# 6Lackiu/EMplanner_Carla

Hardware: AMD Instinct MI355X
Metric: planning cycles/sec (DP+QP, 40x9 S-L lattice, 8 obs) (higher is better)
Workload: dtype f64

## Files before the change

emplanner_carla_amd/csrc/emp_api.hip:

```cpp
#include <stdlib.h>
#include <string.h>

#include <algorithm>
#include <tuple>

#include "emp_context.h"
#ifndef EMP_QP_LDS_PAD
#define EMP_QP_LDS_PAD 0
#endif
#ifndef EMP_EDGE_LDS_PAD
#define EMP_EDGE_LDS_PAD 0
#endif
#include "emp_dp_kernels.h"
#include "emp_st_kernels.h"
#include "emp_st_backend_kernels.h"
#include "emp_tail_kernels.h"
#include "emp_mpc_kernels.h"
#include "emp_rollout_kernels.h"
#include "emp_speed_front_kernels.h"
#include "emp_drive_kernels.h"

namespace emp {
thread_local std::string g_create_error;

// ... 818 lines not shown
static bool qp_reserved_ok(const emp_qp_params* q) { return EMP_DEV_HOOKS || q->reserved == 0; }

static QpDev make_qp_dev(const emp_qp_params* q) {
    QpDev d;
    d.qp = PathQpParams{q->ds, q->w_l, q->w_ddl, q->w_dddl, q->w_centre, q->host_d1, q->host_d2, q->host_w};
    d.obs_length = q->obs_length;
    d.obs_width = q->obs_width;
    d.decimate = q->decimate > 0 ? q->decimate : 1;
    d.midpoint = q->midpoint;
    d.use_qp = q->use_qp;
    d.debug_stage = EMP_DEV_HOOKS ? q->reserved : 0;
    return d;
}

static inline dim3 grid1(int n, int block) { return dim3((unsigned)((n + block - 1) / block)); }
static inline dim3 grid_groups(int B, int per_wave) { return grid1(B, per_wave); }

static int dev_project(emp_ctx* ctx, int B, int max_ref, int max_obs, const double* ref_line, const int* n_ref,
                       const double* origin_xy, const double* start_xy, const double* start_v, const double* start_a,
                       const double* obs_xy, const int* n_obs, double* s_map, double* obs_s, double* obs_l,
                       double* begin_sl, double* start, int obs_cap = -1, const double* dyn = nullptr,
                       int* n_obs_out = nullptr) {
    if (B == 0) return EMP_OK;
    const size_t lds = (size_t)7 * max_ref * sizeof(double);
    if (const int rc = set_lds(ctx, frenet_project_wave_kernel, lds, "reference line too long for the LDS-resident projection kernel")) return rc;
    return launch(ctx, "project", frenet_project_wave_kernel, dim3(B), dim3(64), lds, B, max_ref, max_obs, ref_line, n_ref, origin_xy,
                  start_xy, start_v, start_a, obs_xy, n_obs, s_map, obs_s, obs_l, begin_sl, start, obs_cap < 0 ? max_obs : obs_cap, dyn,
                  n_obs_out);
}

template <typename... A>
static int dev_reference_line(emp_ctx* ctx, const emp_smooth_params* sp, int B, int max_global, A... args) {
    if (B == 0) return EMP_OK;
    const SmoothQpParams sx{sp->w_smooth, sp->w_length, sp->w_ref, sp->x_thre};
    const SmoothQpParams sy{sp->w_smooth, sp->w_length, sp->w_ref, sp->y_thre};
    const size_t lds = (2 * (size_t)kRefLinePoints + 2 * (size_t)BoxRangeQp::words(kRefLinePoints, kRefLinePoints) +
                        (size_t)kRefLinePoints) * sizeof(double);
    if (const int rc = set_lds(ctx, reference_line_wave_kernel, lds, kQpTooLarge)) return rc;
    return launch(ctx, "reference_line", reference_line_wave_kernel, dim3(B), dim3(64), lds, B, max_global, sx, sy, args...);
}

static int dev_cycle_qp(emp_ctx* ctx, int B, int max_pts, int max_obs, const QpDev& Q, const double* dp_s,
                        const double* dp_l, const int* dp_len, const double* obs_s, const double* obs_l,
                        const int* n_obs, const double* start, double* path_s, double* path_l, int* path_len,
                        int* status, CycleSched* cs) {
    if (B == 0) return EMP_OK;
    const int cap = (max_pts + Q.decimate - 1) / Q.decimate;
    const size_t per_group = ((size_t)5 * cap + 4 * (size_t)max_obs + path_qp_words(cap)) * sizeof(double);
    int rc;
    KernelTimer t(ctx, "path_qp");
    const bool pair_form = ctx->opt[EMP_OPT_PATH_QP_FORM] == 1;
    if (cap <= 66 && !pair_form) {
        const int gp = cap <= 34 ? 8 : 16;
        const size_t words = cap <= 26 ? cycle_qp_group_words<8, 3>(cap, max_obs) : cap <= 34 ? cycle_qp_group_words<8, 4>(cap, max_obs)
                                                                                                : cycle_qp_group_words<16, 4>(cap, max_obs);
        const size_t per_wave = (size_t)(64 / gp) * words * sizeof(double) + EMP_QP_LDS_PAD;
        auto kern = cap <= 26 ? cycle_qp_rows_kernel<8, 3> : cap <= 34 ? cycle_qp_rows_kernel<8, 4> : cycle_qp_rows_kernel<16, 4>;
        if ((rc = set_lds(ctx, kern, per_wave, kQpTooLarge))) return rc;
        const int spw = 64 / gp;
        return launch_attaching(ctx, cs, t.stop != nullptr, kern, dim3((B + spw - 1) / spw), dim3(64), per_wave, B, max_pts,
                                max_obs, cap, Q, dp_s, dp_l, dp_len, obs_s, obs_l, n_obs, start, path_s, path_l, path_len, status);
    } else if (cap <= 34) {
        const size_t per_pair = 2 * ((size_t)5 * cap + 4 * (size_t)max_obs + path_qp_words_pair()) * sizeof(double);
        auto kern = cycle_qp_wave_kernel<32>;
        if ((rc = set_lds(ctx, kern, per_pair, kQpTooLarge))) return rc;
        return launch_attaching(ctx, cs, t.stop != nullptr, kern, dim3((B + 1) / 2), dim3(64), per_pair, B, max_pts,
                                max_obs, cap, Q, dp_s, dp_l, dp_len, obs_s, obs_l, n_obs, start, path_s, path_l, path_len, status);
    }
    if ((rc = set_lds(ctx, cycle_qp_wave_kernel<64>, per_group, kQpTooLarge))) return rc;
    return launch_attaching(ctx, cs, t.stop != nullptr, cycle_qp_wave_kernel<64>, dim3(B), dim3(64), per_group, B, max_pts, max_obs, cap,
                            Q, dp_s, dp_l, dp_len, obs_s, obs_l, n_obs, start, path_s, path_l, path_len, status);
}

static int dev_cycle_cartesian(emp_ctx* ctx, int B, int max_ref, int max_pts, int path_cap, const emp_smooth_params* sp,
                               const double* ref_line, const double* s_map, const int* n_ref, const double* begin_sl,
                               const double* path_s, const double* path_l, const int* path_len, double* traj,
                               int* traj_len, int* status) {
    if (B == 0) return EMP_OK;
    const SmoothQpParams sx{sp->w_smooth, sp->w_length, sp->w_ref, sp->x_thre};
    const SmoothQpParams sy{sp->w_smooth, sp->w_length, sp->w_ref, sp->y_thre};
    const int cap = path_cap + 1;
    const size_t lds = ((size_t)max_ref + 3 * (size_t)cap + 2 * (size_t)BoxRangeQp::words(cap, cap)) * sizeof(double);
    const bool wave_form = ctx->opt[EMP_OPT_CARTESIAN_FORM] == 1;
    if (cap <= 64 && !wave_form) {
        const int spw = cap <= 32 ? 4 : 2;
        const size_t lds4 = ((size_t)spw * ((size_t)max_ref + 5 * (size_t)cap) + 2 * (size_t)BoxRangeQp::words(cap, cap)) * sizeof(double);
        auto k4 = cap <= 24 ? cycle_cartesian_rows_kernel<8, 3> : cap <= 32 ? cycle_cartesian_rows_kernel<8, 4> : cycle_cartesian_rows_kernel<16, 4>;
        if (const int rc = set_lds(ctx, k4, lds4, kQpTooLarge)) return rc;
        const int force_fb = ctx->opt[EMP_OPT_SMOOTH_FORCE_FALLBACK] ? 1 : 0;
        return launch(ctx, "to_cartesian", k4, dim3((B + spw - 1) / spw), dim3(64), lds4, B, max_ref, max_pts, cap, sx, sy, ref_line,
                      s_map, n_ref, begin_sl, path_s, path_l, path_len, traj, traj_len, status, force_fb);
    }
    auto kern = cap > 32 ? cycle_cartesian_wave_kernel_wide : cycle_cartesian_wave_kernel_narrow;
    if (const int rc = set_lds(ctx, kern, lds, kQpTooLarge)) return rc;
    return launch(ctx, "to_cartesian", kern, dim3(B), dim3(64), lds, B, max_ref, max_pts, cap, sx, sy, ref_line, s_map, n_ref,
                  begin_sl, path_s, path_l, path_len, traj, traj_len, status);
}

class CycleLane {
  public:
    CycleLane(emp_ctx* c, int m, bool p) : ctx(c), mode(m), pinned(p) {}
    ~CycleLane() {
        if (!ln) return;
        ctx->stream = ctx->main_stream;
        std::swap(ctx->pool, ln->pool);
        ctx->active_lane = -1;
    }

    int begin() {
// ... 2000 lines not shown
```

emplanner_carla_amd/csrc/emp_qp_core.h:

```cpp
#pragma once

#include "emp_core.h"

#ifndef EMP_QP_TRACE
#define EMP_QP_TRACE(...)
#endif

namespace emp {

constexpr int kQpMaxIter = 60;
#ifndef EMP_QP_TAU
#define EMP_QP_TAU(mu) fmax(0.99, 1.0 - (mu))
#endif
EMP_HD double qp_step_fraction(double mu) { return EMP_QP_TAU(mu); }
constexpr int kQpStallIter = 16;
constexpr double kQpStallResidual = 1e-3;

template <int KD>
EMP_HD bool band_chol(double* a, int n) {
    constexpr int W = KD + 1;
    for (int i = 0; i < n; ++i) {
        for (int d = 0; d <= KD && i + d < n; ++d) {
            double sum = a[i * W + d];
            const int j = i + d;
// ... 447 lines not shown
            if (i == 0 || i == n - 1) {
                if (v > ub + tol || v < lb - tol) return 1;
            } else {
                const int t = i - 1;
                Q.c[t * 2 + f] = v;
                Q.lo[t * 2 + f] = lb;
                Q.hi[t * 2 + f] = ub;
            }
        }
    }
    const double ds2 = ds * ds;
    const double a[3] = {1.0 / 6.0, 4.0 / 6.0, 1.0 / 6.0};
    const double b[3] = {1.0 / ds2, -2.0 / ds2, 1.0 / ds2};
    const double jk[4] = {-1.0 / ds2, 3.0 / ds2, -3.0 / ds2, 1.0 / ds2};
    const double wl2 = 2.0 * (prm.w_l + prm.w_centre), wd2 = 2.0 * prm.w_ddl, wj2 = 2.0 * prm.w_dddl;
    for (int m = 0; m < N; ++m) {
        Q.q[m] = 0.0;
        Q.u[m] = 0.0;
        for (int d = 0; d < 4; ++d) Q.P[m * 4 + d] = 0.0;
    }
    auto add = [&](int jp, int jq, double val) {
        const int fp = jp - 3, fq = jq - 3;
        const bool pf = fp >= 0 && fp < N, qf = fq >= 0 && fq < N;
        if (pf && qf) Q.P[fp * 4 + (fq - fp)] += val;
        else if (pf) Q.q[fp] += val * cc[jq];
        else if (qf) Q.q[fq] += val * cc[jp];
    };
    for (int i = 0; i < n; ++i) {
        for (int p = 0; p < 3; ++p)
            for (int r = p; r < 3; ++r) add(i + p, i + r, wl2 * a[p] * a[r] + wd2 * b[p] * b[r]);
        if (i + 1 < n)
            for (int p = 0; p < 4; ++p)
                for (int r = p; r < 4; ++r) add(i + p, i + r, wj2 * jk[p] * jk[r]);
        const double lin = -2.0 * prm.w_centre * ((l_min[i] + l_max[i]) / 2.0);
        for (int p = 0; p < 3; ++p) {
            const int f = i + p - 3;
            if (f >= 0 && f < N) Q.q[f] += lin * a[p];
        }
    }
    return 0;
}

EMP_HD void path_qp_finish(const double* cc, int n, double ds, double* out_l, double* out_dl, double* out_ddl) {
    for (int i = 0; i < n; ++i) {
        out_l[i] = (cc[i] + 4.0 * cc[i + 1] + cc[i + 2]) / 6.0;
        if (out_dl) out_dl[i] = (cc[i + 2] - cc[i]) / (2.0 * ds);
        if (out_ddl) out_ddl[i] = (cc[i] - 2.0 * cc[i + 1] + cc[i + 2]) / (ds * ds);
    }
}

EMP_HD constexpr int path_qp_words_pair() { return 36 + PathRangeQp::words_fast(32, 32); }
EMP_HD constexpr int path_qp_words(int n) { return PathRangeQp::words(n - 4 > 0 ? n - 4 : 0, n - 2 > 0 ? n - 2 : 0) + n + 2; }

EMP_HD int path_qp_solve_scalar(double* mem, const double* l_min, const double* l_max, int n, double l0, double dl0,
                                double ddl0, const PathQpParams& prm, double* out_l, double* out_dl, double* out_ddl,
                                int* iters, double* gi_work = nullptr) {
    *iters = 0;
    if (n < 4) return 2;
    PathRangeQp Q;
    double* cc = mem;
    Q.bind(mem + n + 2, n - 4, n - 2);
    int rc = path_qp_setup(Q, cc, l_min, l_max, n, l0, dl0, ddl0, prm);
    if (rc) return rc;
    if (Q.N > 0) {
        for (int m = 0; m < Q.N * 4; ++m) Q.M[m] = Q.P[m];
        if (!band_chol<3>(Q.M, Q.N)) return 2;
        for (int m = 0; m < Q.N; ++m) Q.u[m] = -Q.q[m];
        band_solve<3>(Q.M, Q.u, Q.N);
        rc = gi_work ? range_qp_gi_scalar(Q, gi_work) : Q.solve_scalar();
        *iters = Q.iters;
        if (rc) return rc;
        for (int m = 0; m < Q.N; ++m) cc[m + 3] = Q.u[m];
    } else {
        for (int t = 0; t < Q.ns; ++t)
            for (int f = 0; f < 2; ++f)
                if (Q.c[t * 2 + f] > Q.hi[t * 2 + f] + 1e-9 || Q.c[t * 2 + f] < Q.lo[t * 2 + f] - 1e-9) return 1;
    }
    path_qp_finish(cc, n, prm.ds, out_l, out_dl, out_ddl);
    return 0;
}

struct SmoothQpParams {
    double w_smooth, w_length, w_ref, thr;
};

EMP_HD void box_qp_forms(BoxRangeQp& Q) {
    Q.off0 = 0;
    Q.g[0][0] = 1.0;
    Q.eps_p = 1e-10;
    Q.eps_mu = 1e-13;
    Q.eps_d_rel = 1e-10;
}

EMP_HD int box_qp_setup(BoxRangeQp& Q, const double* ref, int stride, int m, const SmoothQpParams& prm) {
    if (m < 2 || !(prm.thr > 0.0)) return 2;
    box_qp_forms(Q);
    for (int i = 0; i < m * 3; ++i) Q.P[i] = 0.0;
    for (int i = 0; i < m; ++i) Q.P[i * 3] += 2.0 * prm.w_ref;
    const double d2[3] = {1.0, -2.0, 1.0};
    for (int r = 0; r + 2 < m; ++r)
        for (int p = 0; p < 3; ++p)
            for (int cidx = p; cidx < 3; ++cidx) Q.P[(r + p) * 3 + (cidx - p)] += 2.0 * prm.w_smooth * d2[p] * d2[cidx];
    const double d1[2] = {1.0, -1.0};
    for (int r = 0; r + 1 < m; ++r)
        for (int p = 0; p < 2; ++p)
            for (int cidx = p; cidx < 2; ++cidx) Q.P[(r + p) * 3 + (cidx - p)] += 2.0 * prm.w_length * d1[p] * d1[cidx];
// ... 13 lines not shown
```

emplanner_carla_amd/csrc/emp_qp_rows.h:

```cpp
#pragma once

#include "emp_qp_wave.h"

#ifndef EMP_QP_DEBUG_ROWS
#define EMP_QP_DEBUG_ROWS(...)
#endif

namespace emp {

#pragma clang fp contract(fast)

template <int GP, class Op>
__device__ __forceinline__ double oct_reduce(double v, Op op) {
    static_assert(GP == 8 || GP == 16, "groups of 8 or 16 lanes");
    v = op(v, dpp_move<0xB1>(v));
    v = op(v, dpp_move<0x4E>(v));
    v = op(v, dpp_move<0x141>(v));
    if constexpr (GP == 16) v = op(v, dpp_move<0x140>(v));
    return v;
}
template <int GP>
__device__ __forceinline__ double oct_max(double v) { return oct_reduce<GP>(v, [](double a, double b) { return vmax(a, b); }); }
template <int GP>
__device__ __forceinline__ double oct_min(double v) { return oct_reduce<GP>(v, [](double a, double b) { return vmin(a, b); }); }
// ... 110 lines not shown
        for (int r = 0; r < R; ++r) {
            const double y1 = (r >= 1) ? y[r - 1] : p1;
            const double y2 = (r >= 2) ? y[r - 2] : (r == 1 ? p1 : p2);
            const double y3 = (r >= 3) ? y[r - 3] : (r == 2 ? p1 : (r == 1 ? p2 : p3));
            double acc = __builtin_fma(-low[r][1], y1, rhs[r]);
            acc = __builtin_fma(-low[r][2], y2, acc);
            acc = __builtin_fma(-low[r][3], y3, acc);
            y[r] = acc * rinv[r];
        }
    }
    double x[R];
#pragma unroll
    for (int r = 0; r < R; ++r) x[r] = y[r] * rinv[r];
    for (int k = 0; k < steps; ++k) {
        const double q1 = lane_dn1(x[0]), q2 = lane_dn1(x[1]), q3 = lane_dn1(x[2]);
#pragma unroll
        for (int r = R - 1; r >= 0; --r) {
            const double x1 = (r + 1 < R) ? x[r + 1] : q1;
            const double x2 = (r + 2 < R) ? x[r + 2] : (r + 2 == R ? q1 : q2);
            const double x3 = (r + 3 < R) ? x[r + 3] : (r + 3 == R ? q1 : (r + 3 == R + 1 ? q2 : q3));
            double acc = __builtin_fma(-a[r][1], x1, y[r]);
            acc = __builtin_fma(-a[r][2], x2, acc);
            acc = __builtin_fma(-a[r][3], x3, acc);
            x[r] = acc * rinv[r];
        }
    }
#pragma unroll
    for (int r = 0; r < R; ++r) b[r] = x[r];
}

template <int GP, int R>
__device__ int path_qp_solve_rows(PathRangeQp& Q, int gl, bool live, int iter_cap, double* keep) {
    constexpr int F = 2, W = 3;
    const int N = Q.N, ns = Q.ns, rows = ns * F * 2;
    int state = (live && N > 0) ? 1 : 0;
    int iters = 0;
    bool acceptable = false;
    const int base = gl * R;
    const int steps = oct_wave_max<GP>((state == 1) ? (N + R - 1) / R : 0);
    double g[F][W], gg0[W][F], gg1[W - 1][F], gg2[W - 2][F];
#pragma unroll
    for (int f = 0; f < F; ++f) {
#pragma unroll
        for (int p = 0; p < W; ++p) g[f][p] = wave_uniform(Q.g[f][p]);
    }
#pragma unroll
    for (int f = 0; f < F; ++f) {
#pragma unroll
        for (int p = 0; p < W; ++p) gg0[p][f] = wave_uniform(g[f][p] * g[f][p]);
#pragma unroll
        for (int p = 0; p < W - 1; ++p) gg1[p][f] = wave_uniform(g[f][p] * g[f][p + 1]);
        gg2[0][f] = wave_uniform(g[f][0] * g[f][2]);
    }
    unsigned tmask = 0, mmask = 0, uwm = 0, swm = 0, uxm = 0;
#pragma unroll
    for (int r = 0; r < R; ++r) {
        if (live && base + r < ns) tmask |= 1u << r;
        if (live && base + r < N) mmask |= 1u << r;
    }
#pragma unroll
    for (int i = 0; i < R + 2; ++i) {
        const int k = base - 2 + i;
        if (live && k >= 0 && k < N) uwm |= 1u << i;
        if (live && base + i < ns) swm |= 1u << i;
    }
#pragma unroll
    for (int i = 0; i < R + 6; ++i) {
        const int k = base - 3 + i;
        if (live && k >= 0 && k < N) uxm |= 1u << i;
    }
    auto ld = [](const double* a, int i, bool ok) {
        const double raw = a[i];
        return ok ? raw : 0.0;
    };
    auto win = [&](const double* vec, double (&out)[R][F]) {
        double vals[R + 2];
#pragma unroll
        for (int i = 0; i < R + 2; ++i) vals[i] = ld(vec, base - 2 + i, (uwm >> i) & 1u);
#pragma unroll
        for (int r = 0; r < R; ++r) {
#pragma unroll
            for (int f = 0; f < F; ++f) out[r][f] = (g[f][0] * vals[r] + g[f][1] * vals[r + 1]) + g[f][2] * vals[r + 2];
        }
    };
    auto gather = [&](const double* coef, double (&out)[R]) {
        double cw[R + 2][F];
#pragma unroll
        for (int i = 0; i < R + 2; ++i) {
#pragma unroll
            for (int f = 0; f < F; ++f) cw[i][f] = ld(coef, (base + i) * F + f, (swm >> i) & 1u);
        }
#pragma unroll
        for (int r = 0; r < R; ++r) {
            double acc = 0.0;
#pragma unroll
            for (int p = 0; p < W; ++p) {
#pragma unroll
                for (int f = 0; f < F; ++f) acc += g[f][p] * cw[r + 2 - p][f];
            }
            out[r] = acc;
        }
    };
    auto bounds = [&](double (&c_it)[R][F], double (&lo_it)[R][F], double (&hi_it)[R][F]) {
#pragma unroll
        for (int r = 0; r < R; ++r) {
            const bool ok = (tmask >> r) & 1u;
#pragma unroll
            for (int f = 0; f < F; ++f) {
                const double c = Q.c[(base + r) * F + f], lo = Q.lo[(base + r) * F + f], hi = Q.hi[(base + r) * F + f];
                c_it[r][f] = ok ? c : 0.0;
                lo_it[r][f] = ok ? lo : -1e300;
                hi_it[r][f] = ok ? hi : 1e300;
            }
        }
    };

    double su[R][F], sl[R][F], zu[R][F], zl[R][F];
    double pdiag = 0.0, qabs = 0.0;
#pragma unroll
    for (int r = 0; r < R; ++r) {
        const bool ok = (mmask >> r) & 1u;
        pdiag = fmax(pdiag, ld(Q.P, (base + r) * 4, ok));
        qabs = fmax(qabs, fabs(ld(Q.q, base + r, ok)));
    }
    const double pscale = oct_max<GP>(pdiag);
    const double qscale = fmax(oct_max<GP>(qabs), 1.0);
    {
        const double z0 = Q.initial_multiplier(pscale);
        double v[R][F], c_it[R][F], lo_it[R][F], hi_it[R][F];
        bounds(c_it, lo_it, hi_it);
        win(Q.u, v);
        double smin = 1e300;
#pragma unroll
        for (int r = 0; r < R; ++r) {
#pragma unroll
            for (int f = 0; f < F; ++f) {
                zu[r][f] = zl[r][f] = z0;
                su[r][f] = hi_it[r][f] - (c_it[r][f] + v[r][f]);
                sl[r][f] = (c_it[r][f] + v[r][f]) - lo_it[r][f];
                if ((tmask >> r) & 1u) smin = fmin(smin, fmin(su[r][f], sl[r][f]));
            }
        }
        smin = oct_min<GP>(smin);
        const double shift = (smin < 1.0) ? (1.0 - smin) : 0.0;
#pragma unroll
        for (int r = 0; r < R; ++r) {
#pragma unroll
            for (int f = 0; f < F; ++f) {
                su[r][f] += shift;
                sl[r][f] += shift;
            }
        }
    }

    bool restore = false;
    while (__any(state == 1)) {
        const bool run = state == 1;
        bool acc_now = false;
        double rpu[R][F], rpl[R][F], isu[R][F], isl[R][F], izu[R][F], izl[R][F];
        double rp_max = 0.0, zmax = 0.0, mu = 0.0;
        {
            double v[R][F], c_it[R][F], lo_it[R][F], hi_it[R][F];
            bounds(c_it, lo_it, hi_it);
            win(Q.u, v);
#pragma unroll
            for (int r = 0; r < R; ++r) {
                const bool ok = run && ((tmask >> r) & 1u);
#pragma unroll
                for (int f = 0; f < F; ++f) {
                    rpu[r][f] = (c_it[r][f] + v[r][f]) - hi_it[r][f] + su[r][f];
                    rpl[r][f] = lo_it[r][f] - (c_it[r][f] + v[r][f]) + sl[r][f];
                    isu[r][f] = fast_rcp(su[r][f]);
                    isl[r][f] = fast_rcp(sl[r][f]);
                    izu[r][f] = fast_rcp(zu[r][f]);
                    izl[r][f] = fast_rcp(zl[r][f]);
                    if (ok) {
                        Q.tmp[(base + r) * F + f] = zu[r][f] - zl[r][f];
                        Q.wgt[(base + r) * F + f] = zu[r][f] * isu[r][f] + zl[r][f] * isl[r][f];
                        rp_max = vmax(rp_max, vmax_abs(rpu[r][f], rpl[r][f]));
                        zmax = vmax(zmax, vmax(zu[r][f], zl[r][f]));
                        mu += su[r][f] * zu[r][f] + sl[r][f] * zl[r][f];
                    }
                }
            }
        }
        __syncthreads();
        double rd_m[R], fa[R][4], flow[R][4], frinv[R];
        {
            double ux[R + 6], gz[R];
#pragma unroll
            for (int i = 0; i < R + 6; ++i) ux[i] = ld(Q.u, base - 3 + i, (uxm >> i) & 1u);
            gather(Q.tmp, gz);
            double ww[R + 2][F];
#pragma unroll
            for (int i = 0; i < R + 2; ++i) {
#pragma unroll
                for (int f = 0; f < F; ++f) ww[i][f] = ld(Q.wgt, (base + i) * F + f, (swm >> i) & 1u);
            }
            double rd_max = 0.0;
#pragma unroll
            for (int r = 0; r < R; ++r) {
                const bool ok = run && ((mmask >> r) & 1u);
                const int m = base + r;
                double acc = Q.q[m];
#pragma unroll
                for (int d = 0; d < 4; ++d) acc += Q.P[m * 4 + d] * ux[r + 3 + d];
#pragma unroll
                for (int d = 1; d < 4; ++d) acc += ld(Q.P, (m - d) * 4 + d, m - d >= 0) * ux[r + 3 - d];
                rd_m[r] = ok ? acc + gz[r] : 0.0;
                rd_max = vmax_abs(rd_max, rd_m[r]);
                double e0 = Q.P[m * 4 + 0], e1 = Q.P[m * 4 + 1], e2 = Q.P[m * 4 + 2];
                const double e3 = Q.P[m * 4 + 3];
#pragma unroll
                for (int f = 0; f < F; ++f) {
                    e0 += (ww[r + 2][f] * gg0[0][f] + ww[r + 1][f] * gg0[1][f]) + ww[r][f] * gg0[2][f];
                    e1 += ww[r + 2][f] * gg1[0][f] + ww[r + 1][f] * gg1[1][f];
                    e2 += ww[r + 2][f] * gg2[0][f];
                }
                fa[r][0] = ok ? e0 : 0.0;
                fa[r][1] = (ok && m + 1 < N) ? e1 : 0.0;
                fa[r][2] = (ok && m + 2 < N) ? e2 : 0.0;
                fa[r][3] = (ok && m + 3 < N) ? e3 : 0.0;
            }
            rd_max = oct_max<GP>(rd_max);
            rp_max = oct_max<GP>(rp_max);
            zmax = oct_max<GP>(zmax);
            mu = oct_sum<GP>(mu) / (double)rows;
            if (run) {
                const double dscale = fmax(qscale, zmax);
                if (rd_max <= Q.eps_d_rel * dscale && rp_max <= Q.eps_p && mu <= Q.eps_mu) state = 0;
                else if (!(mu == mu) || mu > 1e30 || (iters >= kQpStallIter && rp_max > kQpStallResidual)) state = 2;
                else if (rp_max > kQpStallResidual && zmax > kQpInfeasibleZ * pscale) state = 2;
                else if (iters >= kQpMaxIter || iters >= iter_cap) state = acceptable ? 0 : 2;
                acc_now = rd_max <= 100.0 * Q.eps_d_rel * dscale && rp_max <= 10.0 * Q.eps_p && mu <= 1000.0 * Q.eps_mu;
                if (acc_now) acceptable = true;
                if (state == 1 && acc_now && rp_max <= Q.eps_p && mu <= Q.eps_mu) state = 0;
                if (state == 0 && acceptable && !acc_now) restore = true;
                EMP_QP_DEBUG_ROWS("R it %d rd %.3e rp %.3e mu %.3e zmax %.3e -> state %d acc %d\n", iters, rd_max, rp_max, mu, zmax, state, (int)acceptable);
            }
        }
        if (run && acc_now) {
#pragma unroll
            for (int r = 0; r < R; ++r)
                if ((mmask >> r) & 1u) keep[base + r] = Q.u[base + r];
        }
        if (!__any(state == 1)) break;
        const bool go = state == 1;
#ifdef EMP_QP_PROBE_SKIP_CHOL
        bool okf = true;
#pragma unroll
        for (int r = 0; r < R; ++r) {
            frinv[r] = 1.0 / (fa[r][0] + 1.0);
#pragma unroll
            for (int d = 0; d < 4; ++d) flow[r][d] = 0.0;
        }
#else
        const bool okf = band_chol_rows<GP, R>(fa, frinv, flow, N, gl, go, steps);
#endif
        EMP_QP_DEBUG_ROWS("R    chol ok %d\n", (int)okf);
        if (go && !okf) {
            state = acceptable ? 0 : 2;
            if (acceptable && !acc_now) restore = true;
        }
        const bool go2 = state == 1;
#pragma unroll
        for (int r = 0; r < R; ++r) {
            if (go2 && ((tmask >> r) & 1u)) {
#pragma unroll
                for (int f = 0; f < F; ++f)
                    Q.tmp[(base + r) * F + f] = -(((zu[r][f] * isu[r][f]) * rpu[r][f] - zu[r][f]) - ((zl[r][f] * isl[r][f]) * rpl[r][f] - zl[r][f]));
            }
        }
        __syncthreads();
        double dua[R];
        gather(Q.tmp, dua);
#pragma unroll
        for (int r = 0; r < R; ++r) dua[r] = (go2 && ((mmask >> r) & 1u)) ? (-rd_m[r] + dua[r]) : 0.0;
#ifndef EMP_QP_PROBE_SKIP_SOLVE
        band_solve_rows<R>(fa, frinv, flow, dua, steps);
#endif
#pragma unroll
        for (int r = 0; r < R; ++r)
            if (go2 && ((mmask >> r) & 1u)) Q.dua[base + r] = dua[r];
        __syncthreads();
        double rcu[R][F], rcl[R][F];
        {
            double gda[R][F], dsua[R][F], dsla[R][F], dzua[R][F], dzla[R][F];
            win(Q.dua, gda);
            double ratio = 0.0;
#pragma unroll
            for (int r = 0; r < R; ++r) {
                const bool ok = go2 && ((tmask >> r) & 1u);
#pragma unroll
                for (int f = 0; f < F; ++f) {
                    dsua[r][f] = -rpu[r][f] - gda[r][f];
                    dsla[r][f] = -rpl[r][f] + gda[r][f];
                    dzua[r][f] = -zu[r][f] - (zu[r][f] * isu[r][f]) * dsua[r][f];
                    dzla[r][f] = -zl[r][f] - (zl[r][f] * isl[r][f]) * dsla[r][f];
                    if (ok)
                        ratio = vmax(ratio, vmax(vmax(-dsua[r][f] * isu[r][f], -dsla[r][f] * isl[r][f]),
                                                 vmax(-dzua[r][f] * izu[r][f], -dzla[r][f] * izl[r][f])));
                }
            }
            ratio = oct_max<GP>(ratio);
            const double a_aff = (ratio > 1.0) ? fast_rcp(ratio) : 1.0;
            double mu_aff = 0.0;
#pragma unroll
            for (int r = 0; r < R; ++r) {
                if (go2 && ((tmask >> r) & 1u)) {
#pragma unroll
                    for (int f = 0; f < F; ++f)
                        mu_aff += (su[r][f] + a_aff * dsua[r][f]) * (zu[r][f] + a_aff * dzua[r][f]) +
                                  (sl[r][f] + a_aff * dsla[r][f]) * (zl[r][f] + a_aff * dzla[r][f]);
                }
            }
            mu_aff = oct_sum<GP>(mu_aff) / (double)rows;
            double sigma = (mu > 0.0) ? mu_aff * fast_rcp(mu) : 0.0;
            sigma = sigma * sigma * sigma;
#pragma unroll
            for (int r = 0; r < R; ++r) {
                const bool ok = go2 && ((tmask >> r) & 1u);
#pragma unroll
                for (int f = 0; f < F; ++f) {
                    rcu[r][f] = su[r][f] * zu[r][f] + dsua[r][f] * dzua[r][f] - sigma * mu;
                    rcl[r][f] = sl[r][f] * zl[r][f] + dsla[r][f] * dzla[r][f] - sigma * mu;
                }
                if (ok) {
#pragma unroll
                    for (int f = 0; f < F; ++f)
                        Q.tmp[(base + r) * F + f] = -((zu[r][f] * rpu[r][f] - rcu[r][f]) * isu[r][f] - (zl[r][f] * rpl[r][f] - rcl[r][f]) * isl[r][f]);
                }
            }
        }
        __syncthreads();
        double du[R];
        gather(Q.tmp, du);
#pragma unroll
        for (int r = 0; r < R; ++r) du[r] = (go2 && ((mmask >> r) & 1u)) ? (-rd_m[r] + du[r]) : 0.0;
#ifndef EMP_QP_PROBE_SKIP_SOLVE
        band_solve_rows<R>(fa, frinv, flow, du, steps);
#endif
#pragma unroll
        for (int r = 0; r < R; ++r)
            if (go2 && ((mmask >> r) & 1u)) Q.rhs[base + r] = du[r];
        __syncthreads();
        {
            double gd[R][F], dsu[R][F], dsl[R][F], dzu[R][F], dzl[R][F];
            win(Q.rhs, gd);
            double ratio = 0.0;
#pragma unroll
            for (int r = 0; r < R; ++r) {
                const bool ok = go2 && ((tmask >> r) & 1u);
#pragma unroll
                for (int f = 0; f < F; ++f) {
                    dsu[r][f] = -rpu[r][f] - gd[r][f];
                    dsl[r][f] = -rpl[r][f] + gd[r][f];
                    dzu[r][f] = -(rcu[r][f] + zu[r][f] * dsu[r][f]) * isu[r][f];
                    dzl[r][f] = -(rcl[r][f] + zl[r][f] * dsl[r][f]) * isl[r][f];
                    if (ok)
                        ratio = vmax(ratio, vmax(vmax(-dsu[r][f] * isu[r][f], -dsl[r][f] * isl[r][f]),
                                                 vmax(-dzu[r][f] * izu[r][f], -dzl[r][f] * izl[r][f])));
                }
            }
            ratio = oct_max<GP>(ratio);
            const double tau = qp_step_fraction(mu);
            const double alpha = (ratio > tau) ? tau * fast_rcp(ratio) : 1.0;
            EMP_QP_DEBUG_ROWS("R    alpha %.6e\n", alpha);
            if (go2) {
#pragma unroll
                for (int r = 0; r < R; ++r) {
                    if ((tmask >> r) & 1u) {
#pragma unroll
                        for (int f = 0; f < F; ++f) {
                            su[r][f] += alpha * dsu[r][f];
                            sl[r][f] += alpha * dsl[r][f];
                            zu[r][f] += alpha * dzu[r][f];
                            zl[r][f] += alpha * dzl[r][f];
                        }
                    }
                    if ((mmask >> r) & 1u) Q.u[base + r] = Q.u[base + r] + alpha * du[r];
                }
                ++iters;
            }
        }
        __syncthreads();
    }
    if (restore) {
#pragma unroll
        for (int r = 0; r < R; ++r)
            if ((mmask >> r) & 1u) Q.u[base + r] = keep[base + r];
    }
    __syncthreads();
    Q.iters = iters;
    return state;
}

template <int GP, int R>
__host__ __device__ constexpr int path_qp_words_rows() { return (GP * R + 4) + PathRangeQp::words_fast(GP * R, GP * R); }

template <int GP, int R>
__device__ inline int path_qp_group_rows(double* lds, const double* l_min, const double* l_max, int n, double l0, double dl0,
                                         double ddl0, const PathQpParams& prm, double* out_l, int* iters_out, bool live,
                                         int debug_stage = 0) {
    constexpr int kCc = GP * R + 4;
    const int gl = (threadIdx.x & 63) & (GP - 1);
    *iters_out = 0;
    PathRangeQp Q;
    double* cc = lds;
    const int nn = live ? n : 4;
    Q.bind_fast(lds + kCc, GP * R, GP * R, nn - 4 > 0 ? nn - 4 : 0, nn - 2 > 0 ? nn - 2 : 0);
    int rc = path_qp_setup_group<GP>(Q, cc, l_min, l_max, n, l0, dl0, ddl0, prm, gl, live);
    if (!live) rc = 2;
    if (EMP_DEV_HOOKS && debug_stage == 2) rc = 2;
    __syncthreads();
    bool ok = rc == 0;
    const int base = gl * R;
    {
        double fa[R][4], flow[R][4], frinv[R], b0[R];
        const bool act = ok && Q.N > 0;
        const int steps = oct_wave_max<GP>(act ? (Q.N + R - 1) / R : 0);
#pragma unroll
        for (int r = 0; r < R; ++r) {
            const bool has = act && base + r < Q.N;
#pragma unroll
            for (int d = 0; d < 4; ++d) {
                const double raw = Q.P[(base + r) * 4 + d];
                fa[r][d] = has ? raw : 0.0;
            }
            const double qr = Q.q[base + r];
            b0[r] = has ? -qr : 0.0;
        }
        const bool okc = band_chol_rows<GP, R>(fa, frinv, flow, Q.N, gl, act, steps);
        band_solve_rows<R>(fa, frinv, flow, b0, steps);
#pragma unroll
        for (int r = 0; r < R; ++r)
            if (act && base + r < Q.N) Q.u[base + r] = b0[r];
        if (ok && !okc) rc = 2;
    }
    if (EMP_DEV_HOOKS && debug_stage == 3) rc = 2;
    __syncthreads();
    ok = rc == 0;
    const int cap_it = debug_stage >= 10 ? debug_stage - 10 : 1000;
    const int rs = path_qp_solve_rows<GP, R>(Q, gl, ok && Q.N > 0, cap_it, cc + 3);
    if (ok && Q.N > 0) {
        *iters_out = Q.iters;
        if (rs && (debug_stage < 10 || !EMP_DEV_HOOKS)) rc = rs;
    }
    ok = rc == 0;
    if (ok && Q.N == 0) {
        bool bad = false;
        for (int it = gl; it < Q.ns * 2; it += GP)
            if (Q.c[it] > Q.hi[it] + 1e-9 || Q.c[it] < Q.lo[it] - 1e-9) bad = true;
        if (oct_any<GP>(bad)) rc = 1;
    }
    ok = rc == 0;
    for (int m = gl; m < (ok ? Q.N : 0); m += GP) cc[m + 3] = Q.u[m];
    __syncthreads();
    for (int i = gl; i < (ok ? n : 0); i += GP) out_l[i] = (cc[i] + 4.0 * cc[i + 1] + cc[i + 2]) / 6.0;
    __syncthreads();
    return rc;
}

#pragma clang fp contract(off)

}
```

emplanner_carla_amd/csrc/emp_tail_kernels.h:

```cpp
#pragma once

#include <hip/hip_runtime.h>

#include "emp_core.h"
#include "emp_frenet_core.h"
#include "emp_qp_core.h"
#include "emp_qp_wave.h"
#include "emp_qp_rows.h"
#include "emp_smooth_rows.h"

namespace emp {

constexpr int kStDpInfeasible = 1, kStSOutOfRange = 2, kStBoundIndex = 4, kStQpFailed = 8, kStSmoothFailed = 16,
              kStTruncated = 32;

struct QpDev {
    PathQpParams qp;
    double obs_length, obs_width;
    int decimate, midpoint, use_qp;
    int debug_stage;
};

template <int CTRL, int ROW_MASK>
__device__ __forceinline__ void prefix_min_step(double& d, int& li) {
// ... 455 lines not shown

__device__ inline int frenet_path_to_xy(const double* line, const double* s_map, int P, double begin_s, double begin_l,
                                        const double* path_s, const double* path_l, int n, double* target_xy,
                                        int cap, bool* s_error, bool* trunc) {
    *s_error = false;
    *trunc = false;
    int idx = 0, m = 0;
    Node pr;
    if (!proj_point(line, s_map, P, begin_s, &idx, &pr)) {
        *s_error = true;
        return 0;
    }
    target_xy[0] = pr.x + begin_l * (-sin(pr.theta));
    target_xy[1] = pr.y + begin_l * cos(pr.theta);
    m = 1;
    for (int i = 0; i < n; ++i) {
        const double s = path_s[i];
        if (s > s_map[P - 1]) break;
        if (!proj_point(line, s_map, P, s, &idx, &pr)) {
            *s_error = true;
            return m;
        }
        if (m >= cap) {
            *trunc = true;
            break;
        }
        target_xy[2 * m] = pr.x + path_l[i] * (-sin(pr.theta));
        target_xy[2 * m + 1] = pr.y + path_l[i] * cos(pr.theta);
        ++m;
    }
    return m;
}

__global__ void path_to_xy_kernel(int B, int max_ref, int max_pts, const double* __restrict__ ref_line,
                                  const double* __restrict__ s_map, const int* __restrict__ n_ref,
                                  const double* __restrict__ begin_sl, const double* __restrict__ path_s,
                                  const double* __restrict__ path_l, const int* __restrict__ n_pts,
                                  double* __restrict__ target_xy, int* __restrict__ n_out, int* __restrict__ status) {
    const int b = blockIdx.x * blockDim.x + threadIdx.x;
    if (b >= B) return;
    const int P = min(max(n_ref[b], 0), max_ref);
    const int n = min(max(n_pts[b], 0), max_pts);
    bool s_err, trunc;
    const int m = frenet_path_to_xy(ref_line + (size_t)b * max_ref * 4, s_map + (size_t)b * max_ref, P,
                                    begin_sl[2 * b], begin_sl[2 * b + 1], path_s + (size_t)b * max_pts,
                                    path_l + (size_t)b * max_pts, n, target_xy + (size_t)b * (max_pts + 1) * 2,
                                    max_pts + 1, &s_err, &trunc);
    n_out[b] = m;
    status[b] = (s_err ? kStSOutOfRange : 0) | (trunc ? kStTruncated : 0);
}

template <int G, int R = 0>
__host__ __device__ constexpr int cycle_qp_group_words(int cap, int max_obs) {
    if (R > 0) return (path_qp_words_rows<(R > 0 ? G : 8), (R > 0 ? R : 3)>() + (4 * max_obs <= 4 * G * R ? 0 : 4 * max_obs)) | 1;
    return 5 * cap + 4 * max_obs + (G == 32 ? path_qp_words_pair() : path_qp_words(cap));
}
template <int G, int R = 0>
__device__ __forceinline__ void cycle_qp_body(int B, int max_pts, int max_obs, int cap, const QpDev& Q,
                                                           const double* __restrict__ dp_s,
                                                           const double* __restrict__ dp_l,
                                                           const int* __restrict__ dp_len,
                                                           const double* __restrict__ obs_s,
                                                           const double* __restrict__ obs_l,
                                                           const int* __restrict__ n_obs,
                                                           const double* __restrict__ start,
                                                           double* __restrict__ path_s, double* __restrict__ path_l,
                                                           int* __restrict__ path_len, int* __restrict__ status) {
    extern __shared__ __attribute__((aligned(16))) double lds_all[];
    __builtin_amdgcn_s_setprio(EMP_PRIO_BACK);
    constexpr int GPW = 64 / G;
    const int lane = threadIdx.x & 63, grp = lane / G, gl = lane & (G - 1);
    const int b = blockIdx.x * GPW + grp;
    const bool present = b < B;
    static_assert(R == 0 || G == 8 || G == 16, "the rows solver runs on groups of 8 or 16 lanes");
    const int per_group = cycle_qp_group_words<G, R>(cap, max_obs);
    double* lds = lds_all + (size_t)grp * per_group;
    const size_t o = (size_t)(present ? b : 0) * max_pts;
    double* sd = lds;
    double *ld, *lmin, *lmax, *ql, *otab, *qmem;
    if constexpr (R > 0) {
        constexpr int capN = G * R, capS = G * R, kCc = G * R + 4;
        qmem = lds;
        double* qbase = qmem + kCc;
        ql = qbase + capN * 4 + capN * 2;
        sd = qbase + capN * 4 + capN * 4 + capS * 2 * 3;
        ld = sd + cap;
        lmin = ld + cap;
        lmax = lmin + cap;
        otab = 4 * max_obs <= 4 * capN ? qbase : qmem + path_qp_words_rows<G, R>();
    } else {
        ld = sd + cap;
        lmin = ld + cap;
        lmax = lmin + cap;
        ql = lmax + cap;
        otab = ql + cap;
        qmem = otab + 4 * max_obs;
    }
#ifdef EMP_QP_PROBE_EMPTY
    if (Q.debug_stage == 4) return;
#endif
    const int ne = present ? dp_len[b] : 0;
    const int dec = Q.decimate > 0 ? Q.decimate : 1;
    const int n = (ne + dec - 1) / dec;
    const int st = present ? status[b] : 0;
    int fail = 0;
    if (present && (n > cap || n + (Q.midpoint ? 1 : 0) > max_pts || n < 1)) fail = kStTruncated;
    bool live = present && !fail;
    for (int i = gl; i < (live ? n : 0); i += G) {
        sd[i] = dp_s[o + (size_t)i * dec];
        ld[i] = dp_l[o + (size_t)i * dec];
    }
    __syncthreads();
#ifdef EMP_QP_PROBE_EMPTY
    if (Q.debug_stage == 5) return;
#endif
    if (Q.use_qp) {
        const int nob = live ? min(max(n_obs[b], 0), max_obs) : 0;
        bool bad = false;
        for (int k = gl; k < nob; k += G) {
            const double os = obs_s[(size_t)b * max_obs + k], ol = obs_l[(size_t)b * max_obs + k];
            int lo, hi, centre;
            argmin_abs3(sd, n, os - Q.obs_length / 2.0, os + Q.obs_length / 2.0, os, &lo, &hi, &centre);
            lo += 2;
            hi += 2;
            const bool below = ld[centre] < ol;
            otab[4 * k + 0] = (double)lo;
            otab[4 * k + 1] = (double)hi;
            otab[4 * k + 2] = below ? 1.0 : 0.0;
            otab[4 * k + 3] = below ? ol - Q.obs_width / 2.0 : ol + Q.obs_width / 2.0;
            if (lo <= hi && hi >= n) bad = true;
        }
        if (group_any<G>(bad) && live) {
            fail = kStBoundIndex;
            live = false;
        }
        __syncthreads();
        {
            constexpr int T = R > 0 ? R + 1 : (G == 64 ? 4 : 2);
            const int nn = live ? n : 0;
            double a[T], c[T];
#pragma unroll
            for (int t = 0; t < T; ++t) {
// ... 604 lines not shown
```

Baseline: 18.04 million.

## Pad QP rows LDS layout with guard bands to drop per-access bounds masks

```diff
diff --git a/emplanner_carla_amd/csrc/emp_api.hip b/emplanner_carla_amd/csrc/emp_api.hip
--- a/emplanner_carla_amd/csrc/emp_api.hip
+++ b/emplanner_carla_amd/csrc/emp_api.hip
@@ -894,9 +894,8 @@
     const bool pair_form = ctx->opt[EMP_OPT_PATH_QP_FORM] == 1;
     if (cap <= 66 && !pair_form) {
         const int gp = cap <= 34 ? 8 : 16;
-        const size_t words = cap <= 26 ? cycle_qp_group_words<8, 3>(cap, max_obs) : cap <= 34 ? cycle_qp_group_words<8, 4>(cap, max_obs)
-                                                                                                : cycle_qp_group_words<16, 4>(cap, max_obs);
-        const size_t per_wave = (size_t)(64 / gp) * words * sizeof(double) + EMP_QP_LDS_PAD;
+        const size_t per_wave = (cap <= 26 ? PathQpRowsLayout<8, 3>::wave_bytes(max_obs) : cap <= 34 ? PathQpRowsLayout<8, 4>::wave_bytes(max_obs)
+                                                                                          : PathQpRowsLayout<16, 4>::wave_bytes(max_obs)) + EMP_QP_LDS_PAD;
         auto kern = cap <= 26 ? cycle_qp_rows_kernel<8, 3> : cap <= 34 ? cycle_qp_rows_kernel<8, 4> : cycle_qp_rows_kernel<16, 4>;
         if ((rc = set_lds(ctx, kern, per_wave, kQpTooLarge))) return rc;
         const int spw = 64 / gp;
diff --git a/emplanner_carla_amd/csrc/emp_qp_core.h b/emplanner_carla_amd/csrc/emp_qp_core.h
--- a/emplanner_carla_amd/csrc/emp_qp_core.h
+++ b/emplanner_carla_amd/csrc/emp_qp_core.h
@@ -523,6 +523,48 @@
 EMP_HD constexpr int path_qp_words_pair() { return 36 + PathRangeQp::words_fast(32, 32); }
 EMP_HD constexpr int path_qp_words(int n) { return PathRangeQp::words(n - 4 > 0 ? n - 4 : 0, n - 2 > 0 ? n - 2 : 0) + n + 2; }
 
+template <int GP, int R>
+struct PathQpRowsLayout {
+    static constexpr int C = GP * R;
+    static constexpr int kBelowU = 3, kAboveU = 3, kBelowStep = 2, kAboveStation = 2, kRowsAboveP = 3;
+    static constexpr int cc = 0;
+    static constexpr int P = cc + C + 4 + kRowsAboveP * 4;
+    static constexpr int q = P + C * 4;
+    static constexpr int u = q + C + kBelowU;
+    static constexpr int dua = u + C + kAboveU;
+    static constexpr int rhs = dua + C + kBelowStep;
+    static constexpr int c = rhs + C;
+    static constexpr int lo = c + C * 2;
+    static constexpr int hi = lo + C * 2;
+    static constexpr int tmp = hi + C * 2;
+    static constexpr int wgt = tmp + C * 2 + kAboveStation * 2;
+    static constexpr int words = wgt + C * 2 + kAboveStation * 2;
+    static constexpr int max_stations = C + 2;
+    static constexpr int result = dua;
+    static constexpr int path = tmp;
+    static constexpr int obstacles = P;
+    static_assert(kAboveU >= kBelowStep, "dua's windows start inside u's upper guard");
+    static_assert(rhs + C - result >= max_stations, "the result fits into dua .. rhs");
+    static_assert(words - path >= 4 * max_stations, "the decimated path and its bounds fit into tmp .. wgt");
+    static constexpr int stride(int max_obs) { return (words + (max_obs <= C ? 0 : 4 * max_obs)) | 1; }
+    static constexpr size_t wave_bytes(int max_obs) { return (size_t)(64 / GP) * stride(max_obs) * sizeof(double); }
+    template <class Fill>
+    static EMP_HD void pad_ranges(int N, int ns, Fill fill) {
+        fill(P - kRowsAboveP * 4, P, 0.0);
+        fill(P + N * 4, P + C * 4, 0.0);
+        fill(q + N, q + C, 0.0);
+        fill(u - kBelowU, u, 0.0);
+        fill(u + N, dua, 0.0);
+        fill(dua + N, rhs, 0.0);
+        fill(rhs + N, rhs + C, 0.0);
+        fill(c + ns * 2, c + C * 2, 0.0);
+        fill(lo + ns * 2, lo + C * 2, -1e300);
+        fill(hi + ns * 2, hi + C * 2, 1e300);
+        fill(tmp + ns * 2, wgt, 0.0);
+        fill(wgt + ns * 2, words, 0.0);
+    }
+};
+
 EMP_HD int path_qp_solve_scalar(double* mem, const double* l_min, const double* l_max, int n, double l0, double dl0,
                                 double ddl0, const PathQpParams& prm, double* out_l, double* out_dl, double* out_ddl,
                                 int* iters, double* gi_work = nullptr) {
diff --git a/emplanner_carla_amd/csrc/emp_qp_rows.h b/emplanner_carla_amd/csrc/emp_qp_rows.h
--- a/emplanner_carla_amd/csrc/emp_qp_rows.h
+++ b/emplanner_carla_amd/csrc/emp_qp_rows.h
@@ -186,31 +186,18 @@
         for (int p = 0; p < W - 1; ++p) gg1[p][f] = wave_uniform(g[f][p] * g[f][p + 1]);
         gg2[0][f] = wave_uniform(g[f][0] * g[f][2]);
     }
-    unsigned tmask = 0, mmask = 0, uwm = 0, swm = 0, uxm = 0;
+    bool tm[R], mm[R], in1[R], in2[R];
 #pragma unroll
     for (int r = 0; r < R; ++r) {
-        if (live && base + r < ns) tmask |= 1u << r;
-        if (live && base + r < N) mmask |= 1u << r;
-    }
-#pragma unroll
-    for (int i = 0; i < R + 2; ++i) {
-        const int k = base - 2 + i;
-        if (live && k >= 0 && k < N) uwm |= 1u << i;
-        if (live && base + i < ns) swm |= 1u << i;
-    }
-#pragma unroll
-    for (int i = 0; i < R + 6; ++i) {
-        const int k = base - 3 + i;
-        if (live && k >= 0 && k < N) uxm |= 1u << i;
-    }
-    auto ld = [](const double* a, int i, bool ok) {
-        const double raw = a[i];
-        return ok ? raw : 0.0;
-    };
+        tm[r] = live && base + r < ns;
+        mm[r] = live && base + r < N;
+        in1[r] = live && base + r + 1 < N;
+        in2[r] = live && base + r + 2 < N;
+    }
     auto win = [&](const double* vec, double (&out)[R][F]) {
         double vals[R + 2];
 #pragma unroll
-        for (int i = 0; i < R + 2; ++i) vals[i] = ld(vec, base - 2 + i, (uwm >> i) & 1u);
+        for (int i = 0; i < R + 2; ++i) vals[i] = vec[base - 2 + i];
 #pragma unroll
         for (int r = 0; r < R; ++r) {
 #pragma unroll
@@ -222,7 +209,7 @@
 #pragma unroll
         for (int i = 0; i < R + 2; ++i) {
 #pragma unroll
-            for (int f = 0; f < F; ++f) cw[i][f] = ld(coef, (base + i) * F + f, (swm >> i) & 1u);
+            for (int f = 0; f < F; ++f) cw[i][f] = coef[(base + i) * F + f];
         }
 #pragma unroll
         for (int r = 0; r < R; ++r) {
@@ -238,13 +225,11 @@
     auto bounds = [&](double (&c_it)[R][F], double (&lo_it)[R][F], double (&hi_it)[R][F]) {
 #pragma unroll
         for (int r = 0; r < R; ++r) {
-            const bool ok = (tmask >> r) & 1u;
 #pragma unroll
             for (int f = 0; f < F; ++f) {
-                const double c = Q.c[(base + r) * F + f], lo = Q.lo[(base + r) * F + f], hi = Q.hi[(base + r) * F + f];
-                c_it[r][f] = ok ? c : 0.0;
-                lo_it[r][f] = ok ? lo : -1e300;
-                hi_it[r][f] = ok ? hi : 1e300;
+                c_it[r][f] = Q.c[(base + r) * F + f];
+                lo_it[r][f] = Q.lo[(base + r) * F + f];
+                hi_it[r][f] = Q.hi[(base + r) * F + f];
             }
         }
     };
@@ -253,9 +238,8 @@
     double pdiag = 0.0, qabs = 0.0;
 #pragma unroll
     for (int r = 0; r < R; ++r) {
-        const bool ok = (mmask >> r) & 1u;
-        pdiag = fmax(pdiag, ld(Q.P, (base + r) * 4, ok));
-        qabs = fmax(qabs, fabs(ld(Q.q, base + r, ok)));
+        pdiag = fmax(pdiag, Q.P[(base + r) * 4]);
+        qabs = fmax(qabs, fabs(Q.q[base + r]));
     }
     const double pscale = oct_max<GP>(pdiag);
     const double qscale = fmax(oct_max<GP>(qabs), 1.0);
@@ -269,10 +253,10 @@
         for (int r = 0; r < R; ++r) {
 #pragma unroll
             for (int f = 0; f < F; ++f) {
-                zu[r][f] = zl[r][f] = z0;
+                zu[r][f] = zl[r][f] = tm[r] ? z0 : 0.0;
                 su[r][f] = hi_it[r][f] - (c_it[r][f] + v[r][f]);
                 sl[r][f] = (c_it[r][f] + v[r][f]) - lo_it[r][f];
-                if ((tmask >> r) & 1u) smin = fmin(smin, fmin(su[r][f], sl[r][f]));
+                smin = fmin(smin, fmin(su[r][f], sl[r][f]));
             }
         }
         smin = oct_min<GP>(smin);
@@ -299,7 +283,6 @@
             win(Q.u, v);
 #pragma unroll
             for (int r = 0; r < R; ++r) {
-                const bool ok = run && ((tmask >> r) & 1u);
 #pragma unroll
                 for (int f = 0; f < F; ++f) {
                     rpu[r][f] = (c_it[r][f] + v[r][f]) - hi_it[r][f] + su[r][f];
@@ -308,7 +291,7 @@
                     isl[r][f] = fast_rcp(sl[r][f]);
                     izu[r][f] = fast_rcp(zu[r][f]);
                     izl[r][f] = fast_rcp(zl[r][f]);
-                    if (ok) {
+                    if (tm[r]) {
                         Q.tmp[(base + r) * F + f] = zu[r][f] - zl[r][f];
                         Q.wgt[(base + r) * F + f] = zu[r][f] * isu[r][f] + zl[r][f] * isl[r][f];
                         rp_max = vmax(rp_max, vmax_abs(rpu[r][f], rpl[r][f]));
@@ -323,25 +306,24 @@
         {
             double ux[R + 6], gz[R];
 #pragma unroll
-            for (int i = 0; i < R + 6; ++i) ux[i] = ld(Q.u, base - 3 + i, (uxm >> i) & 1u);
+            for (int i = 0; i < R + 6; ++i) ux[i] = Q.u[base - 3 + i];
             gather(Q.tmp, gz);
             double ww[R + 2][F];
 #pragma unroll
             for (int i = 0; i < R + 2; ++i) {
 #pragma unroll
-                for (int f = 0; f < F; ++f) ww[i][f] = ld(Q.wgt, (base + i) * F + f, (swm >> i) & 1u);
+                for (int f = 0; f < F; ++f) ww[i][f] = Q.wgt[(base + i) * F + f];
             }
             double rd_max = 0.0;
 #pragma unroll
             for (int r = 0; r < R; ++r) {
-                const bool ok = run && ((mmask >> r) & 1u);
                 const int m = base + r;
                 double acc = Q.q[m];
 #pragma unroll
                 for (int d = 0; d < 4; ++d) acc += Q.P[m * 4 + d] * ux[r + 3 + d];
 #pragma unroll
-                for (int d = 1; d < 4; ++d) acc += ld(Q.P, (m - d) * 4 + d, m - d >= 0) * ux[r + 3 - d];
-                rd_m[r] = ok ? acc + gz[r] : 0.0;
+                for (int d = 1; d < 4; ++d) acc += Q.P[(m - d) * 4 + d] * ux[r + 3 - d];
+                rd_m[r] = mm[r] ? acc + gz[r] : 0.0;
                 rd_max = vmax_abs(rd_max, rd_m[r]);
                 double e0 = Q.P[m * 4 + 0], e1 = Q.P[m * 4 + 1], e2 = Q.P[m * 4 + 2];
                 const double e3 = Q.P[m * 4 + 3];
@@ -351,10 +333,10 @@
                     e1 += ww[r + 2][f] * gg1[0][f] + ww[r + 1][f] * gg1[1][f];
                     e2 += ww[r + 2][f] * gg2[0][f];
                 }
-                fa[r][0] = ok ? e0 : 0.0;
-                fa[r][1] = (ok && m + 1 < N) ? e1 : 0.0;
-                fa[r][2] = (ok && m + 2 < N) ? e2 : 0.0;
-                fa[r][3] = (ok && m + 3 < N) ? e3 : 0.0;
+                fa[r][0] = e0;
+                fa[r][1] = in1[r] ? e1 : 0.0;
+                fa[r][2] = in2[r] ? e2 : 0.0;
+                fa[r][3] = e3;
             }
             rd_max = oct_max<GP>(rd_max);
             rp_max = oct_max<GP>(rp_max);
@@ -376,7 +358,7 @@
         if (run && acc_now) {
 #pragma unroll
             for (int r = 0; r < R; ++r)
-                if ((mmask >> r) & 1u) keep[base + r] = Q.u[base + r];
+                if (mm[r]) keep[base + r] = Q.u[base + r];
         }
         if (!__any(state == 1)) break;
         const bool go = state == 1;
@@ -384,7 +366,7 @@
         bool okf = true;
 #pragma unroll
         for (int r = 0; r < R; ++r) {
-            frinv[r] = 1.0 / (fa[r][0] + 1.0);
+            frinv[r] = (go && mm[r]) ? 1.0 / (fa[r][0] + 1.0) : 1.0;
 #pragma unroll
             for (int d = 0; d < 4; ++d) flow[r][d] = 0.0;
         }
@@ -399,7 +381,7 @@
         const bool go2 = state == 1;
 #pragma unroll
         for (int r = 0; r < R; ++r) {
-            if (go2 && ((tmask >> r) & 1u)) {
+            if (tm[r]) {
 #pragma unroll
                 for (int f = 0; f < F; ++f)
                     Q.tmp[(base + r) * F + f] = -(((zu[r][f] * isu[r][f]) * rpu[r][f] - zu[r][f]) - ((zl[r][f] * isl[r][f]) * rpl[r][f] - zl[r][f]));
@@ -409,13 +391,13 @@
         double dua[R];
         gather(Q.tmp, dua);
 #pragma unroll
-        for (int r = 0; r < R; ++r) dua[r] = (go2 && ((mmask >> r) & 1u)) ? (-rd_m[r] + dua[r]) : 0.0;
+        for (int r = 0; r < R; ++r) dua[r] = (go2 && mm[r]) ? (-rd_m[r] + dua[r]) : 0.0;
 #ifndef EMP_QP_PROBE_SKIP_SOLVE
         band_solve_rows<R>(fa, frinv, flow, dua, steps);
 #endif
 #pragma unroll
         for (int r = 0; r < R; ++r)
-            if (go2 && ((mmask >> r) & 1u)) Q.dua[base + r] = dua[r];
+            if (mm[r]) Q.dua[base + r] = dua[r];
         __syncthreads();
         double rcu[R][F], rcl[R][F];
         {
@@ -424,7 +406,7 @@
             double ratio = 0.0;
 #pragma unroll
             for (int r = 0; r < R; ++r) {
-                const bool ok = go2 && ((tmask >> r) & 1u);
+                const bool ok = tm[r];
 #pragma unroll
                 for (int f = 0; f < F; ++f) {
                     dsua[r][f] = -rpu[r][f] - gda[r][f];
@@ -441,19 +423,17 @@
             double mu_aff = 0.0;
 #pragma unroll
             for (int r = 0; r < R; ++r) {
-                if (go2 && ((tmask >> r) & 1u)) {
-#pragma unroll
-                    for (int f = 0; f < F; ++f)
-                        mu_aff += (su[r][f] + a_aff * dsua[r][f]) * (zu[r][f] + a_aff * dzua[r][f]) +
-                                  (sl[r][f] + a_aff * dsla[r][f]) * (zl[r][f] + a_aff * dzla[r][f]);
-                }
+#pragma unroll
+                for (int f = 0; f < F; ++f)
+                    mu_aff += (su[r][f] + a_aff * dsua[r][f]) * (zu[r][f] + a_aff * dzua[r][f]) +
+                              (sl[r][f] + a_aff * dsla[r][f]) * (zl[r][f] + a_aff * dzla[r][f]);
             }
             mu_aff = oct_sum<GP>(mu_aff) / (double)rows;
             double sigma = (mu > 0.0) ? mu_aff * fast_rcp(mu) : 0.0;
             sigma = sigma * sigma * sigma;
 #pragma unroll
             for (int r = 0; r < R; ++r) {
-                const bool ok = go2 && ((tmask >> r) & 1u);
+                const bool ok = tm[r];
 #pragma unroll
                 for (int f = 0; f < F; ++f) {
                     rcu[r][f] = su[r][f] * zu[r][f] + dsua[r][f] * dzua[r][f] - sigma * mu;
@@ -470,13 +450,13 @@
         double du[R];
         gather(Q.tmp, du);
 #pragma unroll
-        for (int r = 0; r < R; ++r) du[r] = (go2 && ((mmask >> r) & 1u)) ? (-rd_m[r] + du[r]) : 0.0;
+        for (int r = 0; r < R; ++r) du[r] = (go2 && mm[r]) ? (-rd_m[r] + du[r]) : 0.0;
 #ifndef EMP_QP_PROBE_SKIP_SOLVE
         band_solve_rows<R>(fa, frinv, flow, du, steps);
 #endif
 #pragma unroll
         for (int r = 0; r < R; ++r)
-            if (go2 && ((mmask >> r) & 1u)) Q.rhs[base + r] = du[r];
+            if (mm[r]) Q.rhs[base + r] = du[r];
         __syncthreads();
         {
             double gd[R][F], dsu[R][F], dsl[R][F], dzu[R][F], dzl[R][F];
@@ -484,7 +464,7 @@
             double ratio = 0.0;
 #pragma unroll
             for (int r = 0; r < R; ++r) {
-                const bool ok = go2 && ((tmask >> r) & 1u);
+                const bool ok = tm[r];
 #pragma unroll
                 for (int f = 0; f < F; ++f) {
                     dsu[r][f] = -rpu[r][f] - gd[r][f];
@@ -503,7 +483,7 @@
             if (go2) {
 #pragma unroll
                 for (int r = 0; r < R; ++r) {
-                    if ((tmask >> r) & 1u) {
+                    if (tm[r]) {
 #pragma unroll
                         for (int f = 0; f < F; ++f) {
                             su[r][f] += alpha * dsu[r][f];
@@ -512,7 +492,7 @@
                             zl[r][f] += alpha * dzl[r][f];
                         }
                     }
-                    if ((mmask >> r) & 1u) Q.u[base + r] = Q.u[base + r] + alpha * du[r];
+                    if (mm[r]) Q.u[base + r] = Q.u[base + r] + alpha * du[r];
                 }
                 ++iters;
             }
@@ -522,7 +502,7 @@
     if (restore) {
 #pragma unroll
         for (int r = 0; r < R; ++r)
-            if ((mmask >> r) & 1u) Q.u[base + r] = keep[base + r];
+            if (mm[r]) Q.u[base + r] = keep[base + r];
     }
     __syncthreads();
     Q.iters = iters;
@@ -530,19 +510,37 @@
 }
 
 template <int GP, int R>
-__host__ __device__ constexpr int path_qp_words_rows() { return (GP * R + 4) + PathRangeQp::words_fast(GP * R, GP * R); }
+__host__ __device__ constexpr int path_qp_words_rows() { return PathQpRowsLayout<GP, R>::words; }
+
+template <int GP, int R>
+__device__ __forceinline__ void path_qp_pad_rows(double* lds, int N, int ns, int gl) {
+    PathQpRowsLayout<GP, R>::pad_ranges(N, ns, [&](int first, int last, double v) {
+        for (int i = first + gl; i < last; i += GP) lds[i] = v;
+    });
+}
 
 template <int GP, int R>
 __device__ inline int path_qp_group_rows(double* lds, const double* l_min, const double* l_max, int n, double l0, double dl0,
                                          double ddl0, const PathQpParams& prm, double* out_l, int* iters_out, bool live,
                                          int debug_stage = 0) {
-    constexpr int kCc = GP * R + 4;
+    using L = PathQpRowsLayout<GP, R>;
     const int gl = (threadIdx.x & 63) & (GP - 1);
     *iters_out = 0;
     PathRangeQp Q;
-    double* cc = lds;
+    double* cc = lds + L::cc;
     const int nn = live ? n : 4;
-    Q.bind_fast(lds + kCc, GP * R, GP * R, nn - 4 > 0 ? nn - 4 : 0, nn - 2 > 0 ? nn - 2 : 0);
+    Q.N = nn - 4 > 0 ? nn - 4 : 0;
+    Q.ns = nn - 2 > 0 ? nn - 2 : 0;
+    Q.P = lds + L::P;
+    Q.q = lds + L::q;
+    Q.u = lds + L::u;
+    Q.dua = lds + L::dua;
+    Q.rhs = lds + L::rhs;
+    Q.c = lds + L::c;
+    Q.lo = lds + L::lo;
+    Q.hi = lds + L::hi;
+    Q.tmp = lds + L::tmp;
+    Q.wgt = lds + L::wgt;
     int rc = path_qp_setup_group<GP>(Q, cc, l_min, l_max, n, l0, dl0, ddl0, prm, gl, live);
     if (!live) rc = 2;
     if (EMP_DEV_HOOKS && debug_stage == 2) rc = 2;
@@ -572,8 +570,9 @@
         if (ok && !okc) rc = 2;
     }
     if (EMP_DEV_HOOKS && debug_stage == 3) rc = 2;
+    ok = rc == 0;
+    path_qp_pad_rows<GP, R>(lds, ok ? Q.N : 0, ok ? Q.ns : 0, gl);
     __syncthreads();
-    ok = rc == 0;
     const int cap_it = debug_stage >= 10 ? debug_stage - 10 : 1000;
     const int rs = path_qp_solve_rows<GP, R>(Q, gl, ok && Q.N > 0, cap_it, cc + 3);
     if (ok && Q.N > 0) {
diff --git a/emplanner_carla_amd/csrc/emp_tail_kernels.h b/emplanner_carla_amd/csrc/emp_tail_kernels.h
--- a/emplanner_carla_amd/csrc/emp_tail_kernels.h
+++ b/emplanner_carla_amd/csrc/emp_tail_kernels.h
@@ -531,7 +531,7 @@
 
 template <int G, int R = 0>
 __host__ __device__ constexpr int cycle_qp_group_words(int cap, int max_obs) {
-    if (R > 0) return (path_qp_words_rows<(R > 0 ? G : 8), (R > 0 ? R : 3)>() + (4 * max_obs <= 4 * G * R ? 0 : 4 * max_obs)) | 1;
+    if (R > 0) return PathQpRowsLayout<(R > 0 ? G : 8), (R > 0 ? R : 3)>::stride(max_obs);
     return 5 * cap + 4 * max_obs + (G == 32 ? path_qp_words_pair() : path_qp_words(cap));
 }
 template <int G, int R = 0>
@@ -558,15 +558,14 @@
     double* sd = lds;
     double *ld, *lmin, *lmax, *ql, *otab, *qmem;
     if constexpr (R > 0) {
-        constexpr int capN = G * R, capS = G * R, kCc = G * R + 4;
+        using L = PathQpRowsLayout<G, R>;
         qmem = lds;
-        double* qbase = qmem + kCc;
-        ql = qbase + capN * 4 + capN * 2;
-        sd = qbase + capN * 4 + capN * 4 + capS * 2 * 3;
+        ql = qmem + L::result;
+        sd = qmem + L::path;
         ld = sd + cap;
         lmin = ld + cap;
         lmax = lmin + cap;
-        otab = 4 * max_obs <= 4 * capN ? qbase : qmem + path_qp_words_rows<G, R>();
+        otab = qmem + (max_obs <= L::C ? L::obstacles : L::words);
     } else {
         ld = sd + cap;
         lmin = ld + cap;
```

After: 18.27 million (median of 6 runs). 1.3% higher.
